# Sardhendu/ObjectDetection

Measured on NVIDIA B200. Metric: post-backbone detection images/s @1024^2, higher is better.
Workload: dtype f32

## Files before the change

include/odhead.h:

```cpp
#ifndef ODHEAD_H_
#define ODHEAD_H_

#include <stddef.h>
#include <stdint.h>

#ifdef __cplusplus
extern "C" {
#endif

#ifndef DLPACK_DLPACK_H_
#define DLPACK_DLPACK_H_
typedef enum {
  kDLCPU = 1,
  kDLCUDA = 2,
  kDLCUDAHost = 3,
  kDLCUDAManaged = 13
} DLDeviceType;
typedef struct { DLDeviceType device_type; int32_t device_id; } DLDevice;
typedef enum { kDLInt = 0U, kDLUInt = 1U, kDLFloat = 2U, kDLOpaqueHandle = 3U, kDLBfloat = 4U } DLDataTypeCode;
typedef struct { uint8_t code; uint8_t bits; uint16_t lanes; } DLDataType;
typedef struct {
  void* data;
  DLDevice device;
  int32_t ndim;
  DLDataType dtype;
  int64_t* shape;
  int64_t* strides;
  uint64_t byte_offset;
} DLTensor;
#endif

typedef enum {
  OD_OK = 0,
  OD_ERR_NULL = -1,
  OD_ERR_DTYPE = -2,
  OD_ERR_SHAPE = -3,
  OD_ERR_DEVICE = -4,
  OD_ERR_LAYOUT = -5,
  OD_ERR_WORKSPACE = -6,
  OD_ERR_CUDA = -7,
  OD_ERR_PARAM = -8
} od_status;

#if defined(__GNUC__)
#pragma GCC visibility push(default)
#endif

int od_version(void);
const char* od_source_hash(void);
const char* od_strerror(int status);
const char* od_last_error_detail(void);
int64_t od_launch_count(void);

#define OD_MAX_LEVELS 8
#define OD_MAX_RATIOS 8
typedef struct od_anchor_spec {
  int32_t num_levels;
  int32_t num_ratios;
  double scales[OD_MAX_LEVELS];
  double ratios[OD_MAX_RATIOS];
  int32_t fmap_h[OD_MAX_LEVELS];
  int32_t fmap_w[OD_MAX_LEVELS];
  int32_t fmap_stride[OD_MAX_LEVELS];
  int32_t anchor_stride;
  int32_t image_h, image_w;
} od_anchor_spec;

int64_t od_anchor_count(const od_anchor_spec* spec);
int od_gen_anchors(const od_anchor_spec* spec, int normalized, DLTensor* anchors, void* stream);

int od_apply_box_deltas(const DLTensor* boxes, const DLTensor* deltas, DLTensor* out, void* stream);
int od_clip_boxes(const DLTensor* boxes, const DLTensor* window, DLTensor* out, void* stream);
int od_norm_boxes(const DLTensor* boxes, int32_t image_h, int32_t image_w, int32_t tf_float32, DLTensor* out, void* stream);

size_t od_topk_workspace_bytes(int64_t rows, int64_t cols, int64_t k);
int od_topk(const DLTensor* scores, int64_t k, DLTensor* values, DLTensor* indices,
            void* ws, size_t ws_bytes, void* stream);

size_t od_nms_workspace_bytes(int64_t batch, int64_t num_boxes);
int od_nms(const DLTensor* boxes, const DLTensor* scores, const DLTensor* num_valid,
           float iou_threshold, int64_t max_out, DLTensor* keep_idx, DLTensor* num_kept,
           void* ws, size_t ws_bytes, void* stream);

typedef struct od_proposal_params {
  float bbox_stddev[4];
  int32_t pre_nms_limit;
  int32_t post_nms_count;
  float nms_threshold;
} od_proposal_params;

typedef struct od_proposal_debug {
  DLTensor* ix;
  DLTensor* scores;
  DLTensor* bbox_delta;
  DLTensor* anchors;
  DLTensor* anchor_delta;
  DLTensor* anchor_delta_clipped;
  DLTensor* keep_idx;
  DLTensor* num_kept;
} od_proposal_debug;

size_t od_proposal_workspace_bytes(int64_t batch, int64_t num_anchors, const od_proposal_params* p);
int od_proposal_forward(const DLTensor* rpn_class_probs, const DLTensor* rpn_bbox,
                        const DLTensor* anchors, const od_anchor_spec* spec,
                        const od_proposal_params* params, DLTensor* proposals,
                        const od_proposal_debug* debug,
                        void* ws, size_t ws_bytes, void* stream);

size_t od_proposal_levels_workspace_bytes(int64_t batch, int64_t num_anchors, const od_proposal_params* p);
int od_proposal_forward_levels(const DLTensor* const* class_logits, const DLTensor* const* bbox, int32_t num_levels,
                               const DLTensor* anchors, const od_anchor_spec* spec,
                               const od_proposal_params* params, DLTensor* proposals,
                               const od_proposal_debug* debug,
                               void* ws, size_t ws_bytes, void* stream);

int od_pyramid_roi_align_forward(const DLTensor* const* fmaps, int32_t num_levels, int32_t min_level,
                                 const DLTensor* rois, int32_t image_h, int32_t image_w,
                                 int32_t pool_h, int32_t pool_w,
                                 DLTensor* pooled, DLTensor* roi_level, void* stream);
size_t od_pyramid_roi_align_workspace_bytes(void);
size_t od_pyramid_roi_align_workspace_bytes_n(int64_t n_rois);
int od_roi_processing_order(const DLTensor* rois, int32_t image_h, int32_t image_w, int32_t min_level, int32_t num_levels,
                            DLTensor* order, void* stream);
int od_pyramid_roi_align_forward_ordered(const DLTensor* const* fmaps, int32_t num_levels, int32_t min_level,
                                         const DLTensor* rois, int32_t image_h, int32_t image_w,
                                         int32_t pool_h, int32_t pool_w,
                                         DLTensor* pooled, DLTensor* roi_level, const DLTensor* order,
                                         void* ws, size_t ws_bytes, void* stream);
int od_pyramid_roi_align_forward_ws(const DLTensor* const* fmaps, int32_t num_levels, int32_t min_level,
                                    const DLTensor* rois, int32_t image_h, int32_t image_w,
                                    int32_t pool_h, int32_t pool_w,
                                    DLTensor* pooled, DLTensor* roi_level, void* ws, size_t ws_bytes, void* stream);

int od_crop_and_resize(const DLTensor* image, const DLTensor* boxes, const DLTensor* box_ind,
                       int32_t crop_h, int32_t crop_w, float extrapolation_value,
                       DLTensor* out, void* stream);

typedef struct od_target_params {
  int32_t rois_per_image;
  float bbox_stddev[4];
  int32_t mask_h, mask_w;
  int32_t use_mini_mask;
  int32_t mask_layout_hwg;
} od_target_params;

typedef struct od_target_debug {
  DLTensor* iou;
  DLTensor* roi_iou_max;
  DLTensor* pos_indices;
  DLTensor* neg_indices;
  DLTensor* counts;
  DLTensor* sampled_pos;
  DLTensor* sampled_neg;
  DLTensor* gt_assignment;
} od_target_debug;

size_t od_detection_target_workspace_bytes(int64_t batch, int64_t num_proposals, int64_t num_gt);
int od_detection_target_forward(const DLTensor* proposals, const DLTensor* gt_class_ids,
                                const DLTensor* gt_boxes, const DLTensor* perm_pos, const DLTensor* perm_neg,
                                const od_target_params* params,
                                DLTensor* rois, DLTensor* roi_gt_class_ids, DLTensor* roi_gt_box_deltas,
                                const DLTensor* gt_masks, DLTensor* mask_targets,
// ... 81 lines not shown
```

objectdetection_b200/_lib.py:

```python
from __future__ import annotations

import ctypes
import os
from ctypes import POINTER, c_char_p, c_double, c_float, c_int, c_int32, c_int64, c_size_t, c_void_p

import torch
from torch.utils.dlpack import to_dlpack

_HERE = os.path.dirname(os.path.abspath(__file__))
LIB_PATH = os.environ.get("ODHEAD_LIB") or os.path.join(_HERE, "libodhead.so")

OD_MAX_LEVELS = 8
OD_MAX_RATIOS = 8


class OdHeadError(RuntimeError):

    def __init__(self, status: int, message: str):
        super().__init__(message)
        self.status = status


class AnchorSpec(ctypes.Structure):
    _fields_ = [("num_levels", c_int32), ("num_ratios", c_int32),
                ("scales", c_double * OD_MAX_LEVELS), ("ratios", c_double * OD_MAX_RATIOS),
                ("fmap_h", c_int32 * OD_MAX_LEVELS), ("fmap_w", c_int32 * OD_MAX_LEVELS),
                ("fmap_stride", c_int32 * OD_MAX_LEVELS),
                ("anchor_stride", c_int32), ("image_h", c_int32), ("image_w", c_int32)]


class ProposalParams(ctypes.Structure):
    _fields_ = [("bbox_stddev", c_float * 4), ("pre_nms_limit", c_int32), ("post_nms_count", c_int32),
                ("nms_threshold", c_float)]


class ProposalDebug(ctypes.Structure):
    _fields_ = [(n, c_void_p) for n in ("ix", "scores", "bbox_delta", "anchors", "anchor_delta",
                                        "anchor_delta_clipped", "keep_idx", "num_kept")]


class TargetParams(ctypes.Structure):
    _fields_ = [("rois_per_image", c_int32), ("bbox_stddev", c_float * 4), ("mask_h", c_int32), ("mask_w", c_int32),
                ("use_mini_mask", c_int32), ("mask_layout_hwg", c_int32)]


class TargetDebug(ctypes.Structure):
    _fields_ = [(n, c_void_p) for n in ("iou", "roi_iou_max", "pos_indices", "neg_indices", "counts",
                                        "sampled_pos", "sampled_neg", "gt_assignment")]


class RpnTargetParams(ctypes.Structure):
    _fields_ = [("max_rpn_targets", c_int32), ("bbox_stddev", c_double * 4)]


class DetectionParams(ctypes.Structure):
    _fields_ = [("bbox_stddev", c_float * 4), ("min_confidence", c_float), ("nms_threshold", c_float),
                ("max_instances", c_int32)]


class DetectionDebug(ctypes.Structure):
    _fields_ = [(n, c_void_p) for n in ("class_ids", "class_scores", "bbox_delta", "refined_proposals",
                                        "clipped_proposals", "keep_mask", "nms_keep_mask")]


class FrcnnParams(ctypes.Structure):
    _fields_ = [("feat_stride", c_int32), ("image_h", c_int32), ("image_w", c_int32), ("min_box_hw", c_int32),
                ("pre_nms_top_n", c_int32), ("post_nms_top_n", c_int32), ("nms_threshold", c_double),
                ("num_anchors", c_int32), ("base_anchors", c_double * 64)]


_P = c_void_p
SIGNATURES = {
    "od_version": (c_int, []),
    "od_source_hash": (c_char_p, []),
    "od_strerror": (c_char_p, [c_int]),
    "od_last_error_detail": (c_char_p, []),
    "od_launch_count": (c_int64, []),
    "od_anchor_count": (c_int64, [POINTER(AnchorSpec)]),
    "od_gen_anchors": (c_int, [POINTER(AnchorSpec), c_int, _P, _P]),
    "od_apply_box_deltas": (c_int, [_P, _P, _P, _P]),
    "od_clip_boxes": (c_int, [_P, _P, _P, _P]),
    "od_norm_boxes": (c_int, [_P, c_int32, c_int32, c_int32, _P, _P]),
    "od_topk_workspace_bytes": (c_size_t, [c_int64, c_int64, c_int64]),
    "od_topk": (c_int, [_P, c_int64, _P, _P, _P, c_size_t, _P]),
    "od_nms_workspace_bytes": (c_size_t, [c_int64, c_int64]),
    "od_nms": (c_int, [_P, _P, _P, c_float, c_int64, _P, _P, _P, c_size_t, _P]),
    "od_proposal_workspace_bytes": (c_size_t, [c_int64, c_int64, POINTER(ProposalParams)]),
    "od_proposal_forward": (c_int, [_P, _P, _P, POINTER(AnchorSpec), POINTER(ProposalParams), _P,
                                    POINTER(ProposalDebug), _P, c_size_t, _P]),
    "od_proposal_levels_workspace_bytes": (c_size_t, [c_int64, c_int64, POINTER(ProposalParams)]),
    "od_proposal_forward_levels": (c_int, [POINTER(_P), POINTER(_P), c_int32, _P, POINTER(AnchorSpec), POINTER(ProposalParams),
                                           _P, POINTER(ProposalDebug), _P, c_size_t, _P]),
    "od_rpn_loss_workspace_bytes": (c_size_t, [c_int64, c_int64]),
    "od_rpn_loss_forward": (c_int, [_P, _P, _P, _P, _P, _P, _P, _P, c_size_t, _P]),
    "od_mrcnn_loss_forward": (c_int, [_P, _P, _P, _P, _P, _P, _P, _P]),
    "od_pyramid_roi_align_forward": (c_int, [POINTER(_P), c_int32, c_int32, _P, c_int32, c_int32, c_int32, c_int32,
                                             _P, _P, _P]),
    "od_pyramid_roi_align_workspace_bytes": (c_size_t, []),
    "od_pyramid_roi_align_workspace_bytes_n": (c_size_t, [c_int64]),
    "od_pyramid_roi_align_forward_ws": (c_int, [POINTER(_P), c_int32, c_int32, _P, c_int32, c_int32, c_int32, c_int32,
                                                _P, _P, _P, c_size_t, _P]),
    "od_pyramid_roi_align_forward_ordered": (c_int, [POINTER(_P), c_int32, c_int32, _P, c_int32, c_int32, c_int32, c_int32,
                                                     _P, _P, _P, _P, c_size_t, _P]),
    "od_roi_processing_order": (c_int, [_P, c_int32, c_int32, c_int32, c_int32, _P, _P]),
    "od_crop_and_resize": (c_int, [_P, _P, _P, c_int32, c_int32, c_float, _P, _P]),
    "od_detection_target_workspace_bytes": (c_size_t, [c_int64, c_int64, c_int64]),
    "od_detection_target_forward": (c_int, [_P, _P, _P, _P, _P, POINTER(TargetParams), _P, _P, _P, _P, _P,
                                            POINTER(TargetDebug), _P, c_size_t, _P]),
    "od_rpn_target_workspace_bytes": (c_size_t, [c_int64, c_int64, c_int64]),
    "od_rpn_target_forward": (c_int, [_P, _P, _P, _P, _P, POINTER(RpnTargetParams), _P, _P, _P, _P, _P, c_size_t, _P]),
    "od_detection_workspace_bytes": (c_size_t, [c_int64, c_int64, c_int64]),
    "od_detection_forward": (c_int, [_P, _P, _P, _P, POINTER(DetectionParams), _P, POINTER(DetectionDebug), _P,
                                     c_size_t, _P]),
    "od_unmold_detections": (c_int, [_P, _P, _P, _P, _P, _P, _P, _P]),
    "od_frcnn_proposal_workspace_bytes_batch": (c_size_t, [c_int64, c_int64, c_int64, POINTER(FrcnnParams)]),
    "od_frcnn_proposal_workspace_bytes": (c_size_t, [c_int64, c_int64, POINTER(FrcnnParams)]),
    "od_frcnn_proposal_forward": (c_int, [_P, _P, POINTER(FrcnnParams), _P, _P, _P, c_size_t, _P]),
    "od_roi_pool_forward": (c_int, [_P, _P, c_float, c_float, _P, _P]),
}

_lib = None


def lib() -> ctypes.CDLL:
    global _lib
    if _lib is None:
        if not os.path.exists(LIB_PATH):
            raise OdHeadError(-100, f"{LIB_PATH} is missing: the CUDA extension was not built "
                                    "(run `python -m objectdetection_b200.build`); there is no CPU fallback")
        L = ctypes.CDLL(LIB_PATH)
        for name, (res, args) in SIGNATURES.items():
            fn = getattr(L, name)
            fn.restype, fn.argtypes = res, args
        if os.path.isdir(os.path.join(_HERE, "csrc")) and not os.environ.get("ODHEAD_LIB"):
            from .build import source_hash
            have, want = L.od_source_hash().decode(), source_hash()
            if have != want:
                raise OdHeadError(-100, f"{LIB_PATH} is stale (built from sources {have[:12]}, tree has {want[:12]}): "
                                        "run `python -m objectdetection_b200.build`")
        _lib = L
    return _lib


_pyapi = ctypes.pythonapi
_pyapi.PyCapsule_GetPointer.restype = c_void_p
_pyapi.PyCapsule_GetPointer.argtypes = [ctypes.py_object, c_char_p]
_pyapi.PyCapsule_IsValid.restype = c_int
_pyapi.PyCapsule_IsValid.argtypes = [ctypes.py_object, c_char_p]


class DL:

    def __init__(self):
        self._caps = []

    def __call__(self, t):
        if t is None:
            return None
        if not isinstance(t, torch.Tensor):
            raise TypeError(f"expected a torch.Tensor, got {type(t)}")
        cap = to_dlpack(t)
        if not _pyapi.PyCapsule_IsValid(cap, b"dltensor"):
            raise OdHeadError(-101, "torch did not produce a legacy 'dltensor' capsule")
        self._caps.append(cap)
        return _pyapi.PyCapsule_GetPointer(cap, b"dltensor")


def check(status: int, what: str):
# ... 101 lines not shown
```

objectdetection_b200/csrc/detection.cu:

```cuda
#include "nms.cuh"
#include "topk.cuh"

namespace od {

constexpr int kFinThreads = 1024;

struct DetDebugPtrs {
  int32_t* class_ids;
  float* class_scores;
  float4* bbox_delta;
  float4* refined;
  float4* clipped;
  int32_t* keep_mask;
};

__global__ void __launch_bounds__(256)
det_prepare_kernel(const float4* __restrict__ proposals, const float* __restrict__ probs,
                   const float4* __restrict__ bbox, const float4* __restrict__ window, int N, int C, int n_pow2,
                   float4 stddev, float min_conf, int32_t* __restrict__ cls_out, float* __restrict__ score_out,
                   float4* __restrict__ clipped_out, unsigned long long* __restrict__ keys,
                   int32_t* __restrict__ num_valid, DetDebugPtrs dbg) {
  const int lane = threadIdx.x & 31;
  const int64_t slot = ((int64_t)blockIdx.x * blockDim.x + threadIdx.x) >> 5;
  const int b = blockIdx.y;
// ... 34 lines not shown
  }
  if (lane != 0) return;
  if (arg == 0x7fffffff) arg = 0;
  const float score = p[arg];
  const float4 raw = __ldg(&bbox[r * C + arg]);
  const float4 d = make_float4(raw.x * stddev.x, raw.y * stddev.y, raw.z * stddev.z, raw.w * stddev.w);
  const float4 ref = decode_box(proposals[r], d);
  const float4 cl = clip_box(ref, window[b]);
  const bool keep = (arg > 0) && (score > min_conf);
  cls_out[r] = arg;
  score_out[r] = score;
  clipped_out[r] = cl;
  keys[(int64_t)b * n_pow2 + n] =
      keep ? (((unsigned long long)(C - arg) << 48) | ((unsigned long long)score_key(score) << 16) |
              (unsigned long long)(0xFFFFu - (uint32_t)n))
           : (unsigned long long)(0xFFFFu - (uint32_t)n);
  if (dbg.class_ids) dbg.class_ids[r] = arg;
  if (dbg.class_scores) dbg.class_scores[r] = score;
  if (dbg.bbox_delta) dbg.bbox_delta[r] = d;
  if (dbg.refined) dbg.refined[r] = ref;
  if (dbg.clipped) dbg.clipped[r] = cl;
  if (dbg.keep_mask) dbg.keep_mask[r] = keep ? 1 : 0;
}

constexpr int kDetRankThreads = 256;
constexpr int kDetRankMine = 64;
constexpr int kDetRankTile = 1024;
__global__ void __launch_bounds__(kDetRankThreads)
det_rank_gather_kernel(const unsigned long long* __restrict__ keys, const float4* __restrict__ clipped,
                       const int32_t* __restrict__ cls, int N, int n_pow2, unsigned long long* __restrict__ sorted_keys,
                       float4* __restrict__ sorted_boxes, int32_t* __restrict__ group, int32_t* __restrict__ num_valid) {
  __shared__ unsigned long long tile[kDetRankTile];
  __shared__ int32_t partial[kDetRankThreads];
  const int b = blockIdx.y;
  const unsigned long long* in = keys + (int64_t)b * n_pow2;
  const int me = blockIdx.x * kDetRankMine + (threadIdx.x & (kDetRankMine - 1));
  const int part = threadIdx.x / kDetRankMine;
  constexpr int kParts = kDetRankThreads / kDetRankMine;
  const unsigned long long mine = (me < N) ? in[me] : ~0ull;
  int rank = 0;
  for (int t0 = 0; t0 < N; t0 += kDetRankTile) {
    __syncthreads();
    for (int i = threadIdx.x; i < kDetRankTile; i += kDetRankThreads) tile[i] = (t0 + i < N) ? in[t0 + i] : 0ull;
    __syncthreads();
    const unsigned long long* tp = tile + part * (kDetRankTile / kParts);
#pragma unroll 16
    for (int j = 0; j < kDetRankTile / kParts; ++j) rank += (tp[j] > mine) ? 1 : 0;
  }
  partial[threadIdx.x] = rank;
  __syncthreads();
  if (part == 0 && me < N) {
#pragma unroll
    for (int q = 1; q < kParts; ++q) rank += partial[threadIdx.x + q * kDetRankMine];
    const bool valid = (mine >> 48) != 0ull;
    const int n = (int)(0xFFFFu - (uint32_t)(mine & 0xFFFFull));
    OD_DBG_IDX(rank, N);
    sorted_keys[(int64_t)b * n_pow2 + rank] = valid ? mine : 0ull;
    sorted_boxes[(int64_t)b * N + rank] = valid ? clipped[(int64_t)b * N + n] : make_float4(0.f, 0.f, 0.f, 0.f);
    group[(int64_t)b * N + rank] = valid ? cls[(int64_t)b * N + n] : -1;
    if (valid) atomicMax(&num_valid[b], rank + 1);
  }
}

__global__ void det_gather_kernel(const unsigned long long* __restrict__ keys, const float4* __restrict__ clipped,
                                  const int32_t* __restrict__ cls, int N, int n_pow2, float4* __restrict__ sorted_boxes,
                                  int32_t* __restrict__ group, int32_t* __restrict__ num_valid) {
  const int i = blockIdx.x * blockDim.x + threadIdx.x;
  const int b = blockIdx.y;
  if (i >= N) return;
  const unsigned long long k = keys[(int64_t)b * n_pow2 + i];
  const unsigned long long nxt = (i + 1 < n_pow2) ? keys[(int64_t)b * n_pow2 + i + 1] : 0ull;
  const bool valid = (k >> 48) != 0ull, next_valid = (nxt >> 48) != 0ull;
  if (valid && (!next_valid || i == N - 1)) num_valid[b] = i + 1;
  if (valid) {
    const int n = (int)(0xFFFFu - (uint32_t)(k & 0xFFFFull));
    sorted_boxes[(int64_t)b * N + i] = clipped[(int64_t)b * N + n];
    group[(int64_t)b * N + i] = cls[(int64_t)b * N + n];
  } else {
    sorted_boxes[(int64_t)b * N + i] = make_float4(0.f, 0.f, 0.f, 0.f);
    group[(int64_t)b * N + i] = -1;
  }
}

__global__ void __launch_bounds__(kFinThreads)
det_finalize_kernel(const unsigned long long* __restrict__ keys, const int32_t* __restrict__ keep_flag,
                    const int32_t* __restrict__ group, const int32_t* __restrict__ num_valid,
                    const float4* __restrict__ clipped, const int32_t* __restrict__ cls,
                    const float* __restrict__ score, int N, int n_pow2, int M, float* __restrict__ detections,
                    int32_t* __restrict__ nms_keep_mask) {
  extern __shared__ unsigned long long fkeys[];
  int32_t* prefix = reinterpret_cast<int32_t*>(fkeys + n_pow2);
  __shared__ int32_t warp_sums[kFinThreads / 32];
  __shared__ int32_t tile_base;
  const int b = blockIdx.x;
  const int nv = num_valid[b];
  const int tid = threadIdx.x, lane = tid & 31, warp = tid >> 5;
  const int32_t* kf = keep_flag + (int64_t)b * N;
  const int32_t* grp = group + (int64_t)b * N;
  const unsigned long long* kin = keys + (int64_t)b * n_pow2;
  if (tid == 0) tile_base = 0;
  if (nms_keep_mask)
    for (int n = tid; n < N; n += kFinThreads) nms_keep_mask[(int64_t)b * N + n] = 0;
  __syncthreads();
  for (int t0 = 0; t0 < nv; t0 += kFinThreads) {
    const int i = t0 + tid;
    const int f = (i < nv) ? kf[i] : 0;
    int incl = f;
#pragma unroll
    for (int o = 1; o < 32; o <<= 1) {
      const int v = __shfl_up_sync(0xffffffffu, incl, o);
      if (lane >= o) incl += v;
    }
    if (lane == 31) warp_sums[warp] = incl;
    __syncthreads();
    int off = tile_base;
    for (int w = 0; w < warp; ++w) off += warp_sums[w];
    if (i < nv) prefix[i] = off + incl;
    __syncthreads();
    if (tid == kFinThreads - 1) tile_base = off + incl;
    __syncthreads();
  }
  int32_t m = 0;
  for (int t0 = 0; t0 < nv; t0 += kFinThreads) {
    const int i = t0 + tid;
    unsigned long long out = 0ull;
    if (i < nv && kf[i]) {
      const int g = grp[i];
      int lo = 0, hi = i;
      while (lo < hi) {
        const int mid = (lo + hi) >> 1;
        if (grp[mid] < g) lo = mid + 1;
        else hi = mid;
      }
      const int before = (lo > 0) ? prefix[lo - 1] : 0;
      const int rank = prefix[i] - 1 - before;
      if (rank < M) {
        const unsigned long long k = kin[i];
        const uint32_t n = 0xFFFFu - (uint32_t)(k & 0xFFFFull);
        const uint32_t skey = (uint32_t)((k >> 16) & 0xFFFFFFFFull);
        out = ((unsigned long long)skey << 32) | (unsigned long long)(0xFFFFFFFFu - n);
        OD_DBG_IDX(n, N);
        if (nms_keep_mask) nms_keep_mask[(int64_t)b * N + n] = 1;
      }
    }
    const uint32_t bal = __ballot_sync(0xffffffffu, out != 0ull);
    if (lane == 0) warp_sums[warp] = __popc(bal);
    __syncthreads();
    int off = m, total = 0;
    for (int w = 0; w < kFinThreads / 32; ++w) {
      const int c = warp_sums[w];
      if (w < warp) off += c;
      total += c;
    }
    if (out != 0ull) {
      OD_DBG_IDX(off + __popc(bal & ((1u << lane) - 1u)), n_pow2);
      fkeys[off + __popc(bal & ((1u << lane) - 1u))] = out;
    }
    m += total;
    __syncthreads();
  }
  float* det = detections + (int64_t)b * M * 6;
  for (int t = tid; t < m; t += kFinThreads) {
    const unsigned long long mine = fkeys[t];
    int rank = 0;
    for (int j = 0; j < m; ++j) rank += (fkeys[j] > mine) ? 1 : 0;
    if (rank < M) {
      const int n = (int)composite_index(mine);
// ... 215 lines not shown
```

objectdetection_b200/csrc/nms.cu:

```cuda
#include "nms.cuh"
#include "tma.cuh"
#include "topk.cuh"

namespace od {

constexpr int kMaskColTiles = 4;
constexpr int kMaskThreads = 256;
constexpr int kMaskGroups = kMaskThreads / 64;

template <bool FAST>
__global__ void __launch_bounds__(kMaskThreads)
nms_mask_kernel(const float4* __restrict__ boxes, const int32_t* __restrict__ num_valid,
                const int32_t* __restrict__ group, int K, int W, int rb_begin, float thr, int max_out,
                const int32_t* __restrict__ scan_state, int state_stride, int Ws, unsigned long long* __restrict__ mask,
                unsigned long long* __restrict__ diagT) {
  pdl_prologue();
  const int rb = rb_begin + blockIdx.y, b = blockIdx.z;
  const int cb0 = rb + blockIdx.x * kMaskColTiles;
  const int n = num_valid ? min(num_valid[b], K) : K;
  if (cb0 * 64 >= n) return;
  if (scan_state && scan_state[(int64_t)b * state_stride] >= max_out) return;
  __shared__ float4 cbox[kMaskColTiles * 64];
  __shared__ float carea[kMaskColTiles * 64];
  __shared__ int32_t cgrp[kMaskColTiles * 64];
// ... 12 lines not shown
  const int i = rb * 64 + r;
  const bool row_ok = i < n;
  const CBox my = canon_box(row_ok ? bx[i] : make_float4(0.f, 0.f, 0.f, 0.f));
  const int32_t g = (group && row_ok) ? group[(int64_t)b * K + i] : 0;
#pragma unroll
  for (int ct = 0; ct < kMaskColTiles / kMaskGroups; ++ct) {
    const int tile = half + kMaskGroups * ct;
    const int cb = cb0 + tile;
    if (cb * 64 >= n) break;
    unsigned long long bits = 0ull;
    const float4* cbp = cbox + tile * 64;
    const float* cap = carea + tile * 64;
    const int32_t* cgp = cgrp + tile * 64;
    if (FAST) {
      uint32_t cand_lo = 0u, cand_hi = 0u;
#pragma unroll
      for (int jj = 31; jj >= 0; --jj) {
        const float4 c = cbp[jj];
        const uint32_t sgn = __float_as_uint(c.x - my.ymax) & __float_as_uint(my.ymin - c.z) &
                             __float_as_uint(c.y - my.xmax) & __float_as_uint(my.xmin - c.w);
        cand_lo = __funnelshift_l(sgn, cand_lo, 1);
      }
#pragma unroll
      for (int jj = 31; jj >= 0; --jj) {
        const float4 c = cbp[32 + jj];
        const uint32_t sgn = __float_as_uint(c.x - my.ymax) & __float_as_uint(my.ymin - c.z) &
                             __float_as_uint(c.y - my.xmax) & __float_as_uint(my.xmin - c.w);
        cand_hi = __funnelshift_l(sgn, cand_hi, 1);
      }
      unsigned long long m = ((unsigned long long)cand_hi << 32) | cand_lo;
      if (cb == rb) m &= (r == 63) ? 0ull : ~((2ull << r) - 1ull);
      while (m) {
        const int jj = __ffsll((long long)m) - 1;
        m &= m - 1ull;
        const float4 c = cbp[jj];
        const float ih = f_min(my.ymax, c.z) - f_max(my.ymin, c.x);
        const float iw = f_min(my.xmax, c.w) - f_max(my.xmin, c.y);
        const float inter = f_max(ih, 0.0f) * f_max(iw, 0.0f);
        const bool hit = (inter > 0.0f) && (inter / (my.area + cap[jj] - inter) > thr) && (!group || g == cgp[jj]);
        bits |= (unsigned long long)hit << jj;
      }
    } else {
#pragma unroll 8
      for (int jj = 0; jj < 64; ++jj) {
        const float4 c = cbp[jj];
        CBox o;
        o.ymin = c.x; o.xmin = c.y; o.ymax = c.z; o.xmax = c.w; o.area = cap[jj];
        const bool hit = (cb * 64 + jj < n) && (tf_iou(my, o) > thr) && (!group || g == cgp[jj]);
        bits |= (unsigned long long)hit << jj;
      }
    }
    if (cb == rb) bits &= (r == 63) ? 0ull : ~((2ull << r) - 1ull);
    if (!row_ok) bits = 0ull;
    if (cb != rb) {
      OD_DBG_IDX(cb, Ws);
      if (row_ok) mask[((int64_t)b * K + i) * Ws + cb] = bits;
    } else {
      OD_DBG_IDX(cb, W);
      uint32_t* dt = reinterpret_cast<uint32_t*>(diagT + ((int64_t)b * W + cb) * 64);
      const int warp = (t >> 5) & 1, lane = t & 31;
#pragma unroll 8
      for (int jj = 0; jj < 64; ++jj) {
        const uint32_t bal = __ballot_sync(0xffffffffu, (bits >> jj) & 1ull);
        if (lane == 0) dt[jj * 2 + warp] = bal;
      }
    }
  }
}

constexpr int kScanThreads = 256;
constexpr int kScanMaxSlots = 8;
constexpr int kScanCopyParts = 4;
__device__ __forceinline__ void nb_sync(int id) { asm volatile("bar.sync %0, %1;" ::"r"(id), "n"(kScanThreads) : "memory"); }
__device__ __forceinline__ void nb_sync_n(int id, int n) { asm volatile("bar.sync %0, %1;" ::"r"(id), "r"(n) : "memory"); }
__device__ __forceinline__ void nb_arrive_n(int id, int n) { asm volatile("bar.arrive %0, %1;" ::"r"(id), "r"(n) : "memory"); }
__device__ __forceinline__ void nb_arrive(int id) { asm volatile("bar.arrive %0, %1;" ::"r"(id), "n"(kScanThreads) : "memory"); }
__device__ __forceinline__ void smem_or64(unsigned long long* p, unsigned long long v) {
  uint32_t* h = reinterpret_cast<uint32_t*>(p);
  if ((uint32_t)v) atomicOr(h, (uint32_t)v);
  if ((uint32_t)(v >> 32)) atomicOr(h + 1, (uint32_t)(v >> 32));
}

template <bool STAGED>
__global__ void __launch_bounds__(kScanThreads)
nms_scan_kernel(const unsigned long long* __restrict__ mask, const unsigned long long* __restrict__ diagT,
                const int32_t* __restrict__ num_valid, int K, int W, int Ws, int nslots, int max_out, int c_begin, int c_end,
                int final_round, int32_t* __restrict__ scan_state, int state_stride, int32_t* __restrict__ keep_pos,
                int32_t* __restrict__ num_kept, int32_t* __restrict__ keep_flag) {
  pdl_launch_dependents();
  extern __shared__ __align__(128) unsigned long long smem_u64[];
  const int Wr = (W + 15) & ~15;
  unsigned long long* removed = smem_u64;
  unsigned long long* stage = smem_u64 + Wr;
  const size_t slot_words = (size_t)64 * Ws + 64;
  __shared__ __align__(8) unsigned long long full_bar[kScanMaxSlots];
  __shared__ unsigned long long kept_word;
  __shared__ uint4 pipe_ring[2];
  __shared__ int32_t pipe_out[2];
  const int b = blockIdx.x;
  const int tid = threadIdx.x, lane = tid & 31, warp = tid >> 5;
  for (int w = tid; w < Wr; w += kScanThreads) removed[w] = 0ull;
  if (STAGED && tid == 0) {
    for (int s = 0; s < nslots; ++s) mbar_init(&full_bar[s], 1);
    asm volatile("fence.mbarrier_init.release.cluster;" ::: "memory");
    asm volatile("fence.proxy.async.shared::cta;" ::: "memory");
  }
  pdl_wait();
  const int n = num_valid ? min(num_valid[b], K) : K;
  const int Wn = (n + 63) / 64;
  int32_t* state = scan_state ? scan_state + (int64_t)b * state_stride : nullptr;
  const bool resume = state != nullptr && c_begin > 0;
  const int c_last = min(c_end, Wn);
  if (resume) {
    const unsigned long long* sr = reinterpret_cast<const unsigned long long*>(state + 2);
    for (int w = tid; w < Wr; w += kScanThreads) removed[w] = sr[w];
  } else if (keep_flag) {
    for (int i = tid; i < K; i += kScanThreads) keep_flag[(int64_t)b * K + i] = 0;
  }
  __syncthreads();
  const unsigned long long* mrow = mask + (int64_t)b * K * Ws;
  const unsigned long long* dimg = diagT + (int64_t)b * W * 64;

  int kept_total = resume ? state[0] : 0;
  const int c_first = (kept_total >= max_out) ? c_last : c_begin;
  auto stage_chunk = [&](int c) {
    if (STAGED && tid == kScanThreads - 32 && c < c_last) {
      const int slot = (c - c_first) % nslots;
      unsigned long long* bar = &full_bar[slot];
      unsigned long long* dst = stage + (size_t)slot * slot_words;
      const int rows = min(64, n - c * 64);
      const uint32_t row_bytes = (uint32_t)rows * (uint32_t)Ws * 8u;
      mbar_expect_tx(bar, row_bytes + 512u);
      bulk_g2s(dst, mrow + (size_t)c * 64 * Ws, row_bytes, bar);
      bulk_g2s(dst + (size_t)64 * Ws, dimg + (size_t)c * 64, 512u, bar);
    }
  };
  if (STAGED)
    for (int c = c_first; c < c_first + nslots - 1; ++c) stage_chunk(c);

  int c_waited = c_first - 1;
  if (STAGED) {
    if (warp == 0) {
      uint32_t own_lo = 0u, own_hi = 0u;
      uint2 sup0 = make_uint2(0u, 0u), sup1 = sup0, nx0 = sup0, nx1 = sup0;
      int f_slot = 0;
      uint32_t f_par = 0u;
      auto fetch = [&](int c) {
        mbar_wait(&full_bar[f_slot], f_par);
        c_waited = c;
        const uint2* rows = reinterpret_cast<const uint2*>(stage + (size_t)f_slot * slot_words);
        if (++f_slot == nslots) {
          f_slot = 0;
          f_par ^= 1u;
        }
        const uint2* dt = rows + (size_t)64 * Ws;
        const int wn = min(c + 1, Wn - 1);
        sup0 = dt[lane];
        sup1 = dt[lane + 32];
        nx0 = rows[(size_t)lane * Ws + wn];
        nx1 = rows[(size_t)(lane + 32) * Ws + wn];
      };
      const uint32_t lbit = 1u << lane;
      const uint2* removed2 = reinterpret_cast<const uint2*>(removed);
      int c = c_first;
      if (c < c_last) fetch(c);
      for (; c < c_last; ++c) {
        if (c - c_first >= 2) nb_sync_n(3 + (c & 1), kScanThreads - 32);
// ... 400 lines not shown
    __syncthreads();
  }
  const int done = c - lo;
  if (tid < done) {
    int cum = kept_before;
    for (int i = 0; i <= tid; ++i) cum += __popcll(kb_s[i]);
    sy[lo + tid].keep = kb_s[tid];
    sy[lo + tid].cum = cum;
    st_release(&sy[lo + tid].flag, (final_mine && tid == done - 1) ? 2 : 1);
  }
  for (int i = warp; i < done; i += kWideThreads / 32) {
    int base = kept_before;
    for (int q = 0; q < i; ++q) base += __popcll(kb_s[q]);
    const unsigned long long kept = kb_s[i];
#pragma unroll
    for (int h = 0; h < 2; ++h) {
      const int r = lane + 32 * h;
      if ((kept >> r) & 1ull) {
        const int pos = base + __popcll(kept & ((1ull << r) - 1ull));
        OD_DBG_IDX(pos, max_out);
        OD_DBG_IDX((lo + i) * 64 + r, K);
        if (keep_pos) keep_pos[(int64_t)b * max_out + pos] = (lo + i) * 64 + r;
        if (keep_flag) keep_flag[(int64_t)b * K + (lo + i) * 64 + r] = 1;
      }
    }
  }
  if (final_mine) {
    if (keep_pos)
      for (int j = kept_total + tid; j < max_out; j += kWideThreads) keep_pos[(int64_t)b * max_out + j] = -1;
    if (num_kept && tid == 0) num_kept[b] = kept_total;
  }
}

static int64_t scan_state_stride(int64_t W) { return 2 + 2 * ((W + 15) & ~(int64_t)15); }

size_t nms_sorted_workspace_bytes(int64_t B, int64_t K) {
  const int64_t W = (K + 63) / 64, Ws = nms_mask_stride(K);
  Workspace w(nullptr, 0);
  w.take<unsigned long long>((size_t)(B * K * Ws));
  w.take<unsigned long long>((size_t)(B * W * 64));
  w.take<unsigned long long>((size_t)(B * scan_state_stride(W) / 2 + 1));
  w.take<WideSync>((size_t)(B * W + 1));
  return w.off + 256;
}

static size_t wide_scan_smem(int S, int blocks) {
  return ((size_t)((S + 1) & ~1) + (size_t)64 * S + (size_t)blocks * 64 * S * S) * sizeof(unsigned long long);
}
static int wide_scan_blocks(int S) { return wide_scan_smem(S, 2) <= 200 * 1024 ? 2 : 1; }
static int wide_scan_slice(int64_t B, int W, bool* prefetch) {
  int dev = 0, sms = 0, coop = 0;
  if (cudaGetDevice(&dev) != cudaSuccess || cudaDeviceGetAttribute(&sms, cudaDevAttrMultiProcessorCount, dev) != cudaSuccess ||
      cudaDeviceGetAttribute(&coop, cudaDevAttrCooperativeLaunch, dev) != cudaSuccess || !coop)
    return 0;
  for (int pf = 1; pf >= 0; --pf) {
    int occ = 1;
    if (!pf && cudaFuncSetAttribute(nms_scan_wide_kernel<false>, cudaFuncAttributeMaxDynamicSharedMemorySize,
                                    (int)wide_scan_smem(kWideMaxS, 0)) != cudaSuccess)
      return 0;
    if (!pf && cudaOccupancyMaxActiveBlocksPerMultiprocessor(&occ, nms_scan_wide_kernel<false>, kWideThreads, wide_scan_smem(kWideMaxS, 0)) != cudaSuccess)
      return 0;
    const int64_t per_image = ((int64_t)sms * occ) / B;
    if (per_image < 1) continue;
    int64_t G = (W + 3) / 4;
    if (G > per_image) G = per_image;
    const int S = (int)((W + G - 1) / G);
    if (pf) {
      if (S > kWidePrefetchMaxS) continue;
      const size_t smem = wide_scan_smem(S, wide_scan_blocks(S));
      if (smem > 48 * 1024 &&
          cudaFuncSetAttribute(nms_scan_wide_kernel<true>, cudaFuncAttributeMaxDynamicSharedMemorySize, (int)smem) != cudaSuccess)
        continue;
      if (cudaOccupancyMaxActiveBlocksPerMultiprocessor(&occ, nms_scan_wide_kernel<true>, kWideThreads, smem) != cudaSuccess || occ < 1)
        continue;
    } else if (S > kWideMaxS) {
      continue;
    }
    *prefetch = pf != 0;
    return S;
  }
  return 0;
}

static int scan_round_launch(const unsigned long long* mask, const unsigned long long* diagT, const int32_t* num_valid,
                             int64_t B, int64_t K, int64_t mask_stride, int64_t max_out, int c_begin, int c_end,
                             int final_round, int32_t* scan_state, int32_t* keep_pos, int32_t* num_kept, int32_t* keep_flag,
                             WideSync* wide, cudaStream_t st) {
  const int W = (int)((K + 63) / 64), Ws = (int)mask_stride;
  if (Ws < W) OD_FAIL(OD_ERR_PARAM, "NMS mask stride %d < %d words", Ws, W);
  const size_t plain = (size_t)((W + 15) & ~15) * sizeof(unsigned long long);
  const size_t per_slot = ((size_t)64 * Ws + 64) * sizeof(unsigned long long);
  const size_t kSmemBudget = 200 * 1024;
  const int stride = (int)scan_state_stride(W);
  int nslots = 0;
  bool wide_prefetch = false;
  int wide_S = 0;
  if (W > 0 && Ws % 2 == 0 && reinterpret_cast<uintptr_t>(mask) % 16 == 0 && reinterpret_cast<uintptr_t>(diagT) % 16 == 0 &&
      plain + 2 * per_slot <= kSmemBudget) {
    nslots = (int)((kSmemBudget - plain) / per_slot);
    if (nslots > kScanMaxSlots) nslots = kScanMaxSlots;
    if (W <= 32 && nslots > 4) nslots = 4;
  }
  if (nslots >= 2) {
    const size_t smem = plain + (size_t)nslots * per_slot;
    if (smem > 48 * 1024)
      OD_CUDA(cudaFuncSetAttribute(nms_scan_kernel<true>, cudaFuncAttributeMaxDynamicSharedMemorySize, (int)smem));
    OD_CUDA(launch_pdl(nms_scan_kernel<true>, dim3((unsigned)B), dim3(kScanThreads), smem, st, mask, diagT, num_valid, (int)K, W, Ws, nslots, (int)max_out,
                                                                   c_begin, c_end, final_round, scan_state, stride, keep_pos,
                                                                   num_kept, keep_flag));
  } else if (wide && !scan_state && c_begin == 0 && c_end >= W && W >= 64 && (wide_S = wide_scan_slice(B, W, &wide_prefetch)) > 0) {
    int S = wide_S, Ki = (int)K, mo = (int)max_out;
    const dim3 grid((unsigned)((W + S - 1) / S), (unsigned)B);
    OD_CUDA(cudaMemsetAsync(wide, 0, (size_t)B * W * sizeof(WideSync), st));
    int Wi = W, Wsi = Ws;
    const int blocks = wide_prefetch ? wide_scan_blocks(S) : 0;
    int two = blocks == 2;
    void* args[] = {(void*)&mask, (void*)&diagT, (void*)&num_valid, &Ki, &Wi, &Wsi, &S, &mo, &wide, &keep_pos, &num_kept, &keep_flag, &two};
    OD_CUDA(cudaLaunchCooperativeKernel(wide_prefetch ? (const void*)nms_scan_wide_kernel<true> : (const void*)nms_scan_wide_kernel<false>,
                                        grid, dim3(kWideThreads), args, wide_scan_smem(S, blocks), st));
    OD_LAUNCH_CHECK("nms_scan_wide_kernel");
    return OD_OK;
  } else {
    const size_t smem = plain > 0 ? plain : 128;
    if (smem > 48 * 1024)
      OD_CUDA(cudaFuncSetAttribute(nms_scan_kernel<false>, cudaFuncAttributeMaxDynamicSharedMemorySize, (int)smem));
    nms_scan_kernel<false><<<(unsigned)B, kScanThreads, smem, st>>>(mask, diagT, num_valid, (int)K, W, Ws, 0, (int)max_out, c_begin,
                                                                    c_end, final_round, scan_state, stride, keep_pos, num_kept,
                                                                    keep_flag);
  }
  OD_LAUNCH_CHECK("nms_scan_kernel");
  return OD_OK;
}

int nms_sorted_launch(const float4* boxes, const int32_t* num_valid, const int32_t* group, int64_t B, int64_t K,
                      float thr, int64_t max_out, int32_t* keep_pos, int32_t* num_kept, int32_t* keep_flag,
                      void* ws, size_t ws_bytes, cudaStream_t st) {
  if (B == 0) return OD_OK;
  if (B > 65535) OD_FAIL(OD_ERR_PARAM, "NMS batch %lld > 65535", (long long)B);
  if (K >= (1 << 22)) OD_FAIL(OD_ERR_PARAM, "NMS supports < 4M boxes per image");
  const int W = (int)((K + 63) / 64), Ws = (int)nms_mask_stride(K);
  Workspace w(ws, ws_bytes);
  unsigned long long* mask = w.take<unsigned long long>((size_t)(B * K * Ws));
  unsigned long long* diagT = w.take<unsigned long long>((size_t)(B * W * 64));
  int32_t* state = reinterpret_cast<int32_t*>(w.take<unsigned long long>((size_t)(B * scan_state_stride(W) / 2 + 1)));
  WideSync* wide = w.take<WideSync>((size_t)(B * W + 1));
  if (!ws || !w.ok()) OD_FAIL(OD_ERR_WORKSPACE, "NMS workspace %zu < %zu bytes", ws_bytes, w.off);
  if (K == 0)
    return scan_round_launch(mask, diagT, num_valid, B, K, Ws, max_out, 0, 0, 1, nullptr, keep_pos, num_kept, keep_flag, nullptr, st);
  if (W > 65535) OD_FAIL(OD_ERR_PARAM, "NMS tile grid too large");
  int c1 = (int)((max_out + max_out / 2 + 63) / 64);
  const bool two_rounds = c1 + 8 <= W;
  if (!two_rounds) c1 = W;
  const int stride = (int)scan_state_stride(W);
  for (int round = 0; round < (two_rounds ? 2 : 1); ++round) {
    const int rb0 = round == 0 ? 0 : c1, rb1 = round == 0 ? c1 : W;
    const dim3 grid((unsigned)((W - rb0 + kMaskColTiles - 1) / kMaskColTiles), (unsigned)(rb1 - rb0), (unsigned)B);
    const int32_t* st_in = round == 0 ? nullptr : state;
    if (thr >= 0.0f)
      OD_CUDA(launch_pdl(nms_mask_kernel<true>, grid, dim3(kMaskThreads), 0, st, boxes, num_valid, group, (int)K, W, rb0, thr, (int)max_out, st_in,
                                                           stride, Ws, mask, diagT));
    else
      OD_CUDA(launch_pdl(nms_mask_kernel<false>, grid, dim3(kMaskThreads), 0, st, boxes, num_valid, group, (int)K, W, rb0, thr, (int)max_out, st_in,
                                                            stride, Ws, mask, diagT));
    OD_LAUNCH_CHECK("nms_mask_kernel");
    OD_CHECK(scan_round_launch(mask, diagT, num_valid, B, K, Ws, max_out, rb0, rb1, round == (two_rounds ? 1 : 0),
                               two_rounds ? state : nullptr, keep_pos, num_kept, keep_flag, wide, st));
  }
  return OD_OK;
}

int nms_scan_launch(const unsigned long long* mask, const unsigned long long* diagT, const int32_t* num_valid, int64_t B,
                    int64_t K, int64_t mask_stride, int64_t max_out, int32_t* keep_pos, int32_t* num_kept,
                    int32_t* keep_flag, cudaStream_t st) {
  const int W = (int)((K + 63) / 64);
  return scan_round_launch(mask, diagT, num_valid, B, K, mask_stride, max_out, 0, W, 1, nullptr, keep_pos, num_kept,
                           keep_flag, nullptr, st);
}

__global__ void nms_build_keys_kernel(const float* __restrict__ scores, const int32_t* __restrict__ num_valid, int K,
                                      int64_t n_pow2, unsigned long long* __restrict__ keys) {
  const int64_t i = (int64_t)blockIdx.x * blockDim.x + threadIdx.x;
  const int b = blockIdx.y;
  if (i >= n_pow2) return;
  const int n = num_valid ? min(num_valid[b], K) : K;
  keys[(int64_t)b * n_pow2 + i] = (i < n) ? composite_key(scores[(int64_t)b * K + i], (uint32_t)i) : 0ull;
}
__global__ void nms_gather_sorted_kernel(const float4* __restrict__ boxes, const unsigned long long* __restrict__ keys,
                                         const int32_t* __restrict__ num_valid, int K, int64_t n_pow2,
                                         float4* __restrict__ sorted) {
  const int64_t i = (int64_t)blockIdx.x * blockDim.x + threadIdx.x;
  const int b = blockIdx.y;
  const int n = num_valid ? min(num_valid[b], K) : K;
  if (i >= K) return;
  sorted[(int64_t)b * K + i] =
      (i < n) ? boxes[(int64_t)b * K + composite_index(keys[(int64_t)b * n_pow2 + i])] : make_float4(0.f, 0.f, 0.f, 0.f);
}
__global__ void nms_map_back_kernel(const unsigned long long* __restrict__ keys, int64_t n_pow2, int max_out,
                                    int32_t* __restrict__ keep) {
  const int j = blockIdx.x * blockDim.x + threadIdx.x;
  const int b = blockIdx.y;
  if (j >= max_out) return;
  const int32_t pos = keep[(int64_t)b * max_out + j];
  if (pos >= 0) keep[(int64_t)b * max_out + j] = (int32_t)composite_index(keys[(int64_t)b * n_pow2 + pos]);
}

}

using namespace od;

extern "C" {

size_t od_nms_workspace_bytes(int64_t batch, int64_t num_boxes) {
  Workspace w(nullptr, 0);
  w.take<unsigned long long>((size_t)(batch * next_pow2(num_boxes > 0 ? num_boxes : 1)));
  w.take<float4>((size_t)(batch * num_boxes));
  return w.off + 256 + nms_sorted_workspace_bytes(batch, num_boxes);
}

int od_nms(const DLTensor* boxes, const DLTensor* scores, const DLTensor* num_valid, float iou_threshold,
           int64_t max_out, DLTensor* keep_idx, DLTensor* num_kept, void* ws, size_t ws_bytes, void* stream) {
  cudaStream_t st = static_cast<cudaStream_t>(stream);
  DeviceScope scope;
  OD_CHECK(check_tensor(boxes, "boxes", F32, {kAny, kAny, 4}, 16, scope));
  const int64_t B = boxes->shape[0], K = boxes->shape[1];
  OD_CHECK(check_tensor(scores, "scores", F32, {B, K}, 4, scope));
  if (max_out < 0) OD_FAIL(OD_ERR_SHAPE, "keep_idx: max_out = %lld is negative", (long long)max_out);
  OD_CHECK(check_tensor(keep_idx, "keep_idx", I32, {B, max_out}, 4, scope));
  OD_CHECK(check_opt_tensor(num_valid, "num_valid", I32, {B}, 4, scope));
  OD_CHECK(check_opt_tensor(num_kept, "num_kept", I32, {B}, 4, scope));
  if (B == 0 || max_out == 0) return OD_OK;
  if (!ws) OD_FAIL(OD_ERR_WORKSPACE, "NMS workspace is NULL");
  const int64_t n_pow2 = next_pow2(K > 0 ? K : 1);
  Workspace w(ws, ws_bytes);
  unsigned long long* keys = w.take<unsigned long long>((size_t)(B * n_pow2));
  float4* sorted = w.take<float4>((size_t)(B * K));
  w.off = align_up(w.off, 256);
  if (!w.ok() || ws_bytes < w.off + nms_sorted_workspace_bytes(B, K) - 256)
    OD_FAIL(OD_ERR_WORKSPACE, "NMS workspace %zu bytes too small", ws_bytes);
  const int32_t* nv = dptr<int32_t>(num_valid);
  {
    const dim3 g((unsigned)((n_pow2 + 255) / 256), (unsigned)B);
    nms_build_keys_kernel<<<g, 256, 0, st>>>(dptr<float>(scores), nv, (int)K, n_pow2, keys);
    OD_LAUNCH_CHECK("nms_build_keys_kernel");
  }
  OD_CHECK(sort_u64_desc_launch(keys, B, n_pow2, st));
  if (K > 0) {
    const dim3 g((unsigned)((K + 255) / 256), (unsigned)B);
    nms_gather_sorted_kernel<<<g, 256, 0, st>>>(dptr<float4>(boxes), keys, nv, (int)K, n_pow2, sorted);
    OD_LAUNCH_CHECK("nms_gather_sorted_kernel");
  }
  OD_CHECK(nms_sorted_launch(sorted, nv, nullptr, B, K, iou_threshold, max_out, dptr<int32_t>(keep_idx),
                             dptr<int32_t>(num_kept), nullptr, w.base + w.off, ws_bytes - w.off, st));
  {
    const dim3 g((unsigned)((max_out + 255) / 256), (unsigned)B);
    nms_map_back_kernel<<<g, 256, 0, st>>>(keys, n_pow2, (int)max_out, dptr<int32_t>(keep_idx));
    OD_LAUNCH_CHECK("nms_map_back_kernel");
  }
  return OD_OK;
}

}
```

objectdetection_b200/csrc/roi_align.cu:

```cuda
#include <cuda_bf16.h>

#include <type_traits>

#include "common.cuh"
#include "tma.cuh"

namespace od {

struct __align__(16) RoiMeta {
  const void* base;
  int32_t H, W;
  float in_y0, hs, in_x0, ws;
};

struct LevelTable {
  const void* ptr[OD_MAX_LEVELS];
  int32_t H[OD_MAX_LEVELS];
  int32_t W[OD_MAX_LEVELS];
};

__device__ __forceinline__ int32_t roi_level_of(float4 r, int32_t image_h, int32_t image_w, int32_t min_level,
                                                int32_t max_level) {
  const float h = r.z - r.x;
  const float w = r.w - r.y;
// ... 809 lines not shown
  __shared__ BinInfo s_info[kPoolBins * 4];
  const int32_t t = threadIdx.x;
  const int64_t bin0 = (int64_t)blockIdx.x * kPoolBins;
  const int32_t nb = (int32_t)min((int64_t)kPoolBins, total_bins - bin0);
  const int32_t bins_per_roi = oh * ow;
  for (int32_t i = t; i < nb * 4; i += kBinThreads) {
    const int64_t fb = bin0 + (i >> 2);
    const int64_t roi = fb / bins_per_roi;
    const int32_t ob = (int32_t)(fb - roi * bins_per_roi);
    const int32_t oy = ob / ow, ox = ob - oy * ow;
    bin_table_entry<float>(src, roi, 2 * oy + ((i >> 1) & 1), 2 * ox + (i & 1), false, 2 * oh, 2 * ow, D4, nullptr, &s_taps[i], &s_info[i]);
  }
  __syncthreads();
  const int32_t total = nb * D4;
  float4* __restrict__ o = out + bin0 * D4;
  const float4 zero4 = make_float4(0.f, 0.f, 0.f, 0.f);
  for (int32_t e = t; e < total; e += kBinThreads) {
    const int32_t bin = e / D4;
    const uint32_t c = (uint32_t)(e - bin * D4);
    float4 tl[4], tr[4], bl[4], br[4];
    float xl[4], yl[4];
    uint32_t fl[4];
#pragma unroll
    for (int q = 0; q < 4; ++q) {
      const BinTaps tp = s_taps[bin * 4 + q];
      const BinInfo bi = s_info[bin * 4 + q];
      const float4* __restrict__ base = reinterpret_cast<const float4*>(bi.base_flag & ~(uintptr_t)15);
      fl[q] = (uint32_t)(bi.base_flag & 3u);
      xl[q] = bi.xl;
      yl[q] = bi.yl;
      tl[q] = ldg_f4(base + (tp.tl + c));
      tr[q] = ldg_f4(base + (tp.tr + c));
      bl[q] = ldg_f4(base + (tp.bl + c));
      br[q] = ldg_f4(base + (tp.br + c));
    }
    float4 v[4];
#pragma unroll
    for (int q = 0; q < 4; ++q) {
      const float4 top = lerp4p(tl[q], tr[q], xl[q]);
      const float4 bot = lerp4p(bl[q], br[q], xl[q]);
      v[q] = lerp4p(top, bot, yl[q]);
      if (fl[q] != (uint32_t)kBinSample) v[q] = zero4;
    }
    stg_cs_f4(o + e, max4(max4(max4(v[0], v[1]), v[2]), v[3]));
  }
}

static bool crop_rows_serves(const RoiSource& src, int64_t n_rois, int32_t ph, int32_t pw, int32_t D) {
  const int32_t pmax = ph > pw ? ph : pw;
  if (D != 4 * kRowsD4 || ph > kRowsMaxPool || pw > kRowsMaxWidth || pmax < kRowsMinPool || src.mode > 1) return false;
  return n_rois + 4096 <= 0x7FFFFFFFll;
}

template <typename TMap, typename TOut>
constexpr bool kFp32Pair = std::is_same<TMap, float>::value && std::is_same<TOut, float>::value;
template <typename TMap, typename TOut>
static auto rows_kernel() {
  if constexpr (kFp32Pair<TMap, TOut>)
    return static_cast<void (*)(RoiSource, int64_t, int32_t, int32_t, float, float4*, int32_t*, unsigned int*)>(crop_rows_kernel);
  else
    return &crop_rows_kernel<TMap, TOut>;
}
template <typename TMap, typename TOut, int BINS, int UNROLL, bool POW2, bool ORDERED>
static auto bins_kernel() {
  if constexpr (kFp32Pair<TMap, TOut>) return &crop_bins_kernel<BINS, UNROLL, POW2, ORDERED>;
  else return &crop_bins_kernel<TMap, TOut, BINS, UNROLL, POW2, ORDERED>;
}

template <typename TMap, typename TOut>
static int launch_crop_rows(const RoiSource& src, int64_t n_rois, int32_t ph, int32_t pw, int32_t D, float extrap, void* out,
                            int32_t* level_out, unsigned int* counter, cudaStream_t st) {
  if (!crop_rows_serves(src, n_rois, ph, pw, D)) return 1;
  static bool configured[64] = {false};
  static int sms[64] = {0};
  const auto kernel = rows_kernel<TMap, TOut>();
  int dev = 0;
  OD_CUDA(cudaGetDevice(&dev));
  if (dev < 0 || dev >= 64) OD_FAIL(OD_ERR_DEVICE, "device index %d not supported", dev);
  if (!configured[dev]) {
    OD_CUDA(cudaFuncSetAttribute(kernel, cudaFuncAttributeMaxDynamicSharedMemorySize, (int)kRowsRingBytes));
    configured[dev] = true;
  }
  if (!sms[dev]) OD_CUDA(cudaDeviceGetAttribute(&sms[dev], cudaDevAttrMultiProcessorCount, dev));
  const int64_t grid = n_rois < (int64_t)sms[dev] ? n_rois : (int64_t)sms[dev];
  OD_CUDA(launch_pdl(kernel, dim3((unsigned)grid), dim3((unsigned)(32 * pw + 64)), (size_t)kRowsRingBytes, st, src,
                     n_rois, ph, pw, extrap, static_cast<typename OutUnit<TMap, TOut>::T*>(out), level_out, counter));
  OD_LAUNCH_CHECK("crop_rows_kernel");
  return OD_OK;
}

static int launch_roi_order(const RoiSource& src, int32_t* order_buf, cudaStream_t st) {
  OD_CUDA(launch_pdl(roi_order_kernel, dim3((unsigned)src.batch), dim3(kOrderThreads), 0, st, src.boxes, src.rois_per_image,
                     src.image_h, src.image_w, src.min_level, src.num_levels, order_buf));
  OD_LAUNCH_CHECK("roi_order_kernel");
  return OD_OK;
}

template <typename TMap, typename TOut>
static int launch_crop_bins(RoiSource src, int64_t n_rois, int32_t ph, int32_t pw, int32_t D, float extrap,
                            void* out, int32_t* level_out, cudaStream_t st, unsigned int* counter = nullptr,
                            int32_t* order_buf = nullptr, const int32_t* order_in = nullptr) {
  using Out = typename OutUnit<TMap, TOut>::T;
  if (n_rois == 0) return OD_OK;
  const int32_t D4 = D / MapUnit<TMap>::kCh;
  src.order = nullptr;
  const bool order_ok = src.mode == 0 && D == 4 * kRowsD4 && n_rois <= 0x7FFFFFFFll;
  if (order_ok && order_in) {
    src.order = order_in;
  } else if (order_ok && order_buf && n_rois >= 512 && src.rois_per_image <= kOrderThreads * kOrderPerThread) {
    OD_CHECK(launch_roi_order(src, order_buf, st));
    src.order = order_buf;
  }
  const int64_t bins_per_roi = (int64_t)ph * pw;
  if (bins_per_roi > 0x7FFFFFFFll) OD_FAIL(OD_ERR_PARAM, "pool shape %dx%d too large", ph, pw);
  const int64_t total_bins = n_rois * bins_per_roi;
  for (int l = 0; l < (src.mode == 0 ? src.num_levels : 1); ++l)
    if ((int64_t)src.lt.H[l] * src.lt.W[l] * D4 > 0xFFFFFFFFll)
      OD_FAIL(OD_ERR_PARAM, "one image of level %d exceeds 2^32 16-byte units", l);
  {
    const int rc = launch_crop_rows<TMap, TOut>(src, n_rois, ph, pw, D, extrap, out, level_out, counter, st);
    if (rc != 1) return rc;
  }
  int32_t lg = -1;
  if ((D4 & (D4 - 1)) == 0) {
    lg = 0;
    while ((1 << lg) < D4) ++lg;
  }
  if (lg >= 0 && D4 >= 16) {
    if ((int64_t)64 * D4 > 0x7FFFFFFFll) OD_FAIL(OD_ERR_PARAM, "depth %d too large", D);
    const int64_t grid = (total_bins + kBinBins - 1) / kBinBins;
    if (grid > 0x7FFFFFFFll) OD_FAIL(OD_ERR_PARAM, "too many bins: %lld", (long long)total_bins);
    if (src.order)
      OD_CUDA(launch_pdl(bins_kernel<TMap, TOut, kBinBins, kBinUnroll, true, true>(), dim3((unsigned)grid), dim3(kBinThreads), 0,
          st, src, total_bins, (int32_t)bins_per_roi, ph, pw, D4, lg, extrap, static_cast<Out*>(out), level_out));
    else
      OD_CUDA(launch_pdl(bins_kernel<TMap, TOut, kBinBins, kBinUnroll, true, false>(), dim3((unsigned)grid), dim3(kBinThreads), 0,
          st, src, total_bins, (int32_t)bins_per_roi, ph, pw, D4, lg, extrap, static_cast<Out*>(out), level_out));
  } else {
    constexpr int BINS = 512;
    if ((int64_t)BINS * D4 > 0x7FFFFFFFll) OD_FAIL(OD_ERR_PARAM, "depth %d too large", D);
    const int64_t grid = (total_bins + BINS - 1) / BINS;
    if (grid > 0x7FFFFFFFll) OD_FAIL(OD_ERR_PARAM, "too many bins: %lld", (long long)total_bins);
    const auto kernel = lg >= 0 ? bins_kernel<TMap, TOut, BINS, 2, true, false>() : bins_kernel<TMap, TOut, BINS, 2, false, false>();
    kernel<<<(unsigned)grid, kBinThreads, 0, st>>>(src, total_bins, (int32_t)bins_per_roi, ph, pw, D4, lg, extrap,
                                                   static_cast<Out*>(out), level_out);
  }
  OD_LAUNCH_CHECK("crop_bins_kernel");
  return OD_OK;
}

static DType map_or_out_dtype(const DLTensor* t) {
  return (t && t->dtype.code == kDLBfloat && t->dtype.bits == 16 && t->dtype.lanes == 1) ? BF16 : F32;
}
static int check_bf16_depth(DType map_dt, DType out_dt, int64_t D) {
  if ((map_dt == BF16 || out_dt == BF16) && D % 8)
    OD_FAIL(OD_ERR_SHAPE, "depth %lld must be a multiple of 8 with bfloat16 maps or output", (long long)D);
  return OD_OK;
}
template <typename... Args>
static int launch_crop(DType map_dt, DType out_dt, Args... args) {
  if (map_dt == BF16)
    return out_dt == BF16 ? launch_crop_bins<__nv_bfloat16, __nv_bfloat16>(args...) : launch_crop_bins<__nv_bfloat16, float>(args...);
  return out_dt == BF16 ? launch_crop_bins<float, __nv_bfloat16>(args...) : launch_crop_bins<float, float>(args...);
}

}

// ... 155 lines not shown
```

Baseline: 12230.

## Cap registers in NMS scan and finalize kernels, reserve one SM in crop_rows

Replaces the launch_bounds on the NMS scan and detection finalize kernels with explicit __maxnreg__ caps (96 and 24), changing how many warps can be resident and how much spilling may occur. It moves the scan shared-memory sizing into helper functions and exposes a new API that reports scan smem bytes. It also shrinks the persistent crop_rows grid by one SM, leaving room for an overlapping kernel under PDL. The 24-register cap on finalize risks local-memory spills, and the grid change trims peak throughput of the crop stage.

```diff
diff --git a/include/odhead.h b/include/odhead.h
--- a/include/odhead.h
+++ b/include/odhead.h
@@ -78,6 +78,7 @@
             void* ws, size_t ws_bytes, void* stream);
 
 size_t od_nms_workspace_bytes(int64_t batch, int64_t num_boxes);
+size_t od_nms_scan_smem_bytes(int64_t num_boxes);
 int od_nms(const DLTensor* boxes, const DLTensor* scores, const DLTensor* num_valid,
            float iou_threshold, int64_t max_out, DLTensor* keep_idx, DLTensor* num_kept,
            void* ws, size_t ws_bytes, void* stream);
diff --git a/objectdetection_b200/_lib.py b/objectdetection_b200/_lib.py
--- a/objectdetection_b200/_lib.py
+++ b/objectdetection_b200/_lib.py
@@ -84,6 +84,7 @@
     "od_topk_workspace_bytes": (c_size_t, [c_int64, c_int64, c_int64]),
     "od_topk": (c_int, [_P, c_int64, _P, _P, _P, c_size_t, _P]),
     "od_nms_workspace_bytes": (c_size_t, [c_int64, c_int64]),
+    "od_nms_scan_smem_bytes": (c_size_t, [c_int64]),
     "od_nms": (c_int, [_P, _P, _P, c_float, c_int64, _P, _P, _P, c_size_t, _P]),
     "od_proposal_workspace_bytes": (c_size_t, [c_int64, c_int64, POINTER(ProposalParams)]),
     "od_proposal_forward": (c_int, [_P, _P, _P, POINTER(AnchorSpec), POINTER(ProposalParams), _P,
diff --git a/objectdetection_b200/csrc/detection.cu b/objectdetection_b200/csrc/detection.cu
--- a/objectdetection_b200/csrc/detection.cu
+++ b/objectdetection_b200/csrc/detection.cu
@@ -140,7 +140,7 @@
   }
 }
 
-__global__ void __launch_bounds__(kFinThreads)
+__maxnreg__(24) __global__ void
 det_finalize_kernel(const unsigned long long* __restrict__ keys, const int32_t* __restrict__ keep_flag,
                     const int32_t* __restrict__ group, const int32_t* __restrict__ num_valid,
                     const float4* __restrict__ clipped, const int32_t* __restrict__ cls,
diff --git a/objectdetection_b200/csrc/nms.cu b/objectdetection_b200/csrc/nms.cu
--- a/objectdetection_b200/csrc/nms.cu
+++ b/objectdetection_b200/csrc/nms.cu
@@ -118,7 +118,7 @@
 }
 
 template <bool STAGED>
-__global__ void __launch_bounds__(kScanThreads)
+__maxnreg__(96) __global__ void
 nms_scan_kernel(const unsigned long long* __restrict__ mask, const unsigned long long* __restrict__ diagT,
                 const int32_t* __restrict__ num_valid, int K, int W, int Ws, int nslots, int max_out, int c_begin, int c_end,
                 int final_round, int32_t* __restrict__ scan_state, int state_stride, int32_t* __restrict__ keep_pos,
@@ -685,27 +685,36 @@
   return 0;
 }
 
+constexpr size_t kScanSmemBudget = 200 * 1024;
+static size_t scan_plain_bytes(int W) { return (size_t)((W + 15) & ~15) * sizeof(unsigned long long); }
+static int scan_ring_slots(int W, int Ws) {
+  const size_t plain = scan_plain_bytes(W), per_slot = ((size_t)64 * Ws + 64) * sizeof(unsigned long long);
+  if (W == 0 || Ws % 2 != 0 || plain + 2 * per_slot > kScanSmemBudget) return 0;
+  int nslots = (int)((kScanSmemBudget - plain) / per_slot);
+  if (nslots > kScanMaxSlots) nslots = kScanMaxSlots;
+  if (W <= 32 && nslots > 4) nslots = 4;
+  return nslots;
+}
+static size_t scan_smem_bytes(int W, int Ws, int nslots) {
+  const size_t plain = scan_plain_bytes(W);
+  if (nslots >= 2) return plain + (size_t)nslots * ((size_t)64 * Ws + 64) * sizeof(unsigned long long);
+  return plain > 0 ? plain : 128;
+}
+
 static int scan_round_launch(const unsigned long long* mask, const unsigned long long* diagT, const int32_t* num_valid,
                              int64_t B, int64_t K, int64_t mask_stride, int64_t max_out, int c_begin, int c_end,
                              int final_round, int32_t* scan_state, int32_t* keep_pos, int32_t* num_kept, int32_t* keep_flag,
                              WideSync* wide, cudaStream_t st) {
   const int W = (int)((K + 63) / 64), Ws = (int)mask_stride;
   if (Ws < W) OD_FAIL(OD_ERR_PARAM, "NMS mask stride %d < %d words", Ws, W);
-  const size_t plain = (size_t)((W + 15) & ~15) * sizeof(unsigned long long);
-  const size_t per_slot = ((size_t)64 * Ws + 64) * sizeof(unsigned long long);
-  const size_t kSmemBudget = 200 * 1024;
   const int stride = (int)scan_state_stride(W);
   int nslots = 0;
   bool wide_prefetch = false;
   int wide_S = 0;
-  if (W > 0 && Ws % 2 == 0 && reinterpret_cast<uintptr_t>(mask) % 16 == 0 && reinterpret_cast<uintptr_t>(diagT) % 16 == 0 &&
-      plain + 2 * per_slot <= kSmemBudget) {
-    nslots = (int)((kSmemBudget - plain) / per_slot);
-    if (nslots > kScanMaxSlots) nslots = kScanMaxSlots;
-    if (W <= 32 && nslots > 4) nslots = 4;
-  }
+  if (reinterpret_cast<uintptr_t>(mask) % 16 == 0 && reinterpret_cast<uintptr_t>(diagT) % 16 == 0)
+    nslots = scan_ring_slots(W, Ws);
   if (nslots >= 2) {
-    const size_t smem = plain + (size_t)nslots * per_slot;
+    const size_t smem = scan_smem_bytes(W, Ws, nslots);
     if (smem > 48 * 1024)
       OD_CUDA(cudaFuncSetAttribute(nms_scan_kernel<true>, cudaFuncAttributeMaxDynamicSharedMemorySize, (int)smem));
     OD_CUDA(launch_pdl(nms_scan_kernel<true>, dim3((unsigned)B), dim3(kScanThreads), smem, st, mask, diagT, num_valid, (int)K, W, Ws, nslots, (int)max_out,
@@ -724,7 +733,7 @@
     OD_LAUNCH_CHECK("nms_scan_wide_kernel");
     return OD_OK;
   } else {
-    const size_t smem = plain > 0 ? plain : 128;
+    const size_t smem = scan_smem_bytes(W, Ws, 0);
     if (smem > 48 * 1024)
       OD_CUDA(cudaFuncSetAttribute(nms_scan_kernel<false>, cudaFuncAttributeMaxDynamicSharedMemorySize, (int)smem));
     nms_scan_kernel<false><<<(unsigned)B, kScanThreads, smem, st>>>(mask, diagT, num_valid, (int)K, W, Ws, 0, (int)max_out, c_begin,
@@ -820,6 +829,12 @@
   return w.off + 256 + nms_sorted_workspace_bytes(batch, num_boxes);
 }
 
+size_t od_nms_scan_smem_bytes(int64_t num_boxes) {
+  if (num_boxes < 0 || num_boxes >= (1 << 22)) return 0;
+  const int W = (int)((num_boxes + 63) / 64), Ws = (int)nms_mask_stride(num_boxes);
+  return scan_smem_bytes(W, Ws, scan_ring_slots(W, Ws));
+}
+
 int od_nms(const DLTensor* boxes, const DLTensor* scores, const DLTensor* num_valid, float iou_threshold,
            int64_t max_out, DLTensor* keep_idx, DLTensor* num_kept, void* ws, size_t ws_bytes, void* stream) {
   cudaStream_t st = static_cast<cudaStream_t>(stream);
diff --git a/objectdetection_b200/csrc/roi_align.cu b/objectdetection_b200/csrc/roi_align.cu
--- a/objectdetection_b200/csrc/roi_align.cu
+++ b/objectdetection_b200/csrc/roi_align.cu
@@ -915,7 +915,9 @@
     configured[dev] = true;
   }
   if (!sms[dev]) OD_CUDA(cudaDeviceGetAttribute(&sms[dev], cudaDevAttrMultiProcessorCount, dev));
-  const int64_t grid = n_rois < (int64_t)sms[dev] ? n_rois : (int64_t)sms[dev];
+  const int64_t spare_sms = sms[dev] > 1 ? 1 : 0;
+  const int64_t slots = (int64_t)sms[dev] - spare_sms;
+  const int64_t grid = n_rois < slots ? n_rois : slots;
   OD_CUDA(launch_pdl(kernel, dim3((unsigned)grid), dim3((unsigned)(32 * pw + 64)), (size_t)kRowsRingBytes, st, src,
                      n_rois, ph, pw, extrap, static_cast<typename OutUnit<TMap, TOut>::T*>(out), level_out, counter));
   OD_LAUNCH_CHECK("crop_rows_kernel");
```

After: 12550 (median of 6 runs). 2.6% higher.
